# mx-mark/VideoTransformer-pytorch

Hardware: NVIDIA H100
Metric: clips/sec (BxTx3x224x224) TimeSformer-B fwd+bwd (higher is better)
Workload: dtype bf16

## Files before the change

### videotransformer_pytorch_b200/csrc/vt_attention_mma.cu

```cuda
#include "vt_attention_mma.cuh"

namespace vt {

constexpr int MT = 64;
constexpr int MMA_THREADS = 128;
constexpr float MMA_LOG2E = 1.4426950408889634f;
constexpr float MMA_LN2 = 0.6931471805599453f;

__device__ __forceinline__ void mma16816(float (&c)[4], uint32_t a0, uint32_t a1, uint32_t a2, uint32_t a3, uint32_t b0,
                                         uint32_t b1) {
  asm volatile(
      "mma.sync.aligned.m16n8k16.row.col.f32.bf16.bf16.f32 {%0,%1,%2,%3}, {%4,%5,%6,%7}, {%8,%9}, {%0,%1,%2,%3};"
      : "+f"(c[0]), "+f"(c[1]), "+f"(c[2]), "+f"(c[3])
      : "r"(a0), "r"(a1), "r"(a2), "r"(a3), "r"(b0), "r"(b1));
}
__device__ __forceinline__ uint32_t ld32(const __nv_bfloat16* p) { return *reinterpret_cast<const uint32_t*>(p); }
__device__ __forceinline__ uint32_t smem_addr(const void* p) { return static_cast<uint32_t>(__cvta_generic_to_shared(p)); }
template <int N>
__device__ __forceinline__ void zero(float (&x)[N][4]) {
#pragma unroll
  for (int i = 0; i < N; ++i) x[i][0] = x[i][1] = x[i][2] = x[i][3] = 0.f;
}

__device__ __forceinline__ void cp_async16(void* dst, const void* src, bool ok) {
  asm volatile("cp.async.cg.shared.global [%0], [%1], 16, %2;" ::"r"(smem_addr(dst)), "l"(src), "r"(ok ? 16 : 0) : "memory");
}
__device__ __forceinline__ void cp_async4(void* dst, const void* src, bool ok) {
  asm volatile("cp.async.ca.shared.global [%0], [%1], 4, %2;" ::"r"(smem_addr(dst)), "l"(src), "r"(ok ? 4 : 0) : "memory");
}
__device__ __forceinline__ void cp_async_commit() { asm volatile("cp.async.commit_group;" ::: "memory"); }
template <int N>
__device__ __forceinline__ void cp_async_wait() { asm volatile("cp.async.wait_group %0;" ::"n"(N) : "memory"); }

__device__ __forceinline__ void ldsm_x4(uint32_t (&r)[4], uint32_t a) {
  asm volatile("ldmatrix.sync.aligned.m8n8.x4.shared.b16 {%0,%1,%2,%3}, [%4];" : "=r"(r[0]), "=r"(r[1]), "=r"(r[2]), "=r"(r[3]) : "r"(a));
}
__device__ __forceinline__ void ldsm_x4_t(uint32_t (&r)[4], uint32_t a) {
  asm volatile("ldmatrix.sync.aligned.m8n8.x4.trans.shared.b16 {%0,%1,%2,%3}, [%4];" : "=r"(r[0]), "=r"(r[1]), "=r"(r[2]), "=r"(r[3]) : "r"(a));
}

template <int P>
__device__ __forceinline__ int lane_a(int lane) { return (lane & 15) * P + (lane >> 4) * 8; }
template <int P>
__device__ __forceinline__ int lane_b(int lane) { return ((lane & 7) + (lane >> 4) * 8) * P + ((lane >> 3) & 1) * 8; }

template <int HD>
struct PaddedTile {
  static constexpr int P = HD + 8;
  uint32_t base;
  int la, lb;
  __device__ __forceinline__ explicit PaddedTile(const __nv_bfloat16* t)
      : base(smem_addr(t)), la(2 * lane_a<P>(threadIdx.x & 31)), lb(2 * lane_b<P>(threadIdx.x & 31)) {}
  __device__ __forceinline__ uint32_t a(int r0, int c0) const { return base + (r0 * P + c0) * 2 + la; }
  __device__ __forceinline__ uint32_t b(int n0, int c0) const { return base + (n0 * P + c0) * 2 + lb; }
};

__device__ __forceinline__ int swz(int r, int c) { return r * 64 + ((c ^ (r & 7)) << 3); }
struct SwizzledTile {
  uint32_t base;
  int ar, ak, br, bk;
  __device__ __forceinline__ SwizzledTile(uint32_t operand, int r0) : base(operand + r0 * 128) {
    const int lane = threadIdx.x & 31;
    ar = (lane & 15) * 128; ak = (lane >> 4) ^ (lane & 7);
    br = ((lane & 7) + (lane >> 4) * 8) * 128; bk = ((lane >> 3) & 1) ^ (lane & 7);
  }
  __device__ __forceinline__ uint32_t a(int r0, int c0) const { return base + ar + r0 * 128 + (((c0 >> 3) ^ ak) << 4); }
  __device__ __forceinline__ uint32_t b(int n0, int c0) const { return base + br + n0 * 128 + (((c0 >> 3) ^ bk) << 4); }
};

template <int HD>
__device__ __forceinline__ void stage_rows(__nv_bfloat16* dst, const __nv_bfloat16* src, long long rs, int r0, int limit) {
#pragma unroll
  for (int i = threadIdx.x; i < MT * HD / 8; i += MMA_THREADS) {
    const int r = i / (HD / 8), c = (i % (HD / 8)) * 8;
    const bool ok = r0 + r < limit;
    cp_async16(dst + r * (HD + 8) + c, ok ? src + (long long)(r0 + r) * rs + c : src, ok);
  }
}
template <int HD, class DO2>
__device__ __forceinline__ float row_delta(bool ok, int half, DO2 dO2, const __nv_bfloat16* orow) {
  float d = 0.f;
  if (ok) {
#pragma unroll 4
    for (int c = half * (HD / 2); c < (half + 1) * (HD / 2); c += 2) {
      const float2 g = unpack_bf16x2(dO2(c));
      const float2 o = unpack_bf16x2(ld32(orow + c));
      d = fmaf(g.x, o.x, fmaf(g.y, o.y, d));
    }
  }
  return d + __shfl_xor_sync(0xffffffffu, d, 1);
}
template <int HD>
__device__ __forceinline__ void stage_row_stats(float* lse_s, float* del_s, const __nv_bfloat16* dOs, const __nv_bfloat16* orow,
                                                long long o_rs, const float* lrow, int r0, int limit, float* delta_out) {
  const int r = threadIdx.x >> 1, half = threadIdx.x & 1;
  const bool ok = r0 + r < limit;
  const __nv_bfloat16* g = dOs + r * (HD + 8);
  const float d = row_delta<HD>(ok, half, [=](int c) { return ld32(g + c); }, orow + r * o_rs);
  if (half == 0) {
    del_s[r] = d;
    lse_s[r] = ok ? lrow[r] * MMA_LOG2E : INFINITY;
    if (ok && delta_out) delta_out[r0 + r] = d;
  }
}


template <int KC, class Tile>
__device__ __forceinline__ void load_a(uint32_t (&f)[KC][4], const Tile& t, int r0) {
#pragma unroll
  for (int kc = 0; kc < KC; ++kc) ldsm_x4(f[kc], t.a(r0, kc * 16));
}

template <int HD>
struct FwdAcc {
  float o[HD / 8][4];
  float m0 = -INFINITY, m1 = -INFINITY, l0 = 0.f, l1 = 0.f;
  __device__ __forceinline__ FwdAcc() { zero(o); }
};

template <int HD, class Tile>
__device__ __forceinline__ void fwd_tile(FwdAcc<HD>& f, const uint32_t (&qa)[HD / 16][4], const Tile& K, const Tile& V, int k0,
                                         int N, float c) {
  constexpr int NB = HD / 8, KC = HD / 16;
  const int t = threadIdx.x & 3;
  float s[8][4];
  zero(s);
#pragma unroll
  for (int nb = 0; nb < 8; nb += 2) {
    if (k0 + nb * 8 >= N) break;
    const bool hi = k0 + nb * 8 + 8 < N;
#pragma unroll
    for (int kc = 0; kc < KC; ++kc) {
      uint32_t kf[4];
      ldsm_x4(kf, K.b(nb * 8, kc * 16));
      mma16816(s[nb], qa[kc][0], qa[kc][1], qa[kc][2], qa[kc][3], kf[0], kf[1]);
      if (hi) mma16816(s[nb + 1], qa[kc][0], qa[kc][1], qa[kc][2], qa[kc][3], kf[2], kf[3]);
    }
  }
  float mx0 = -INFINITY, mx1 = -INFINITY;
#pragma unroll
  for (int nb = 0; nb < 8; ++nb) {
#pragma unroll
    for (int e = 0; e < 4; ++e) {
      const int key = k0 + nb * 8 + 2 * t + (e & 1);
      const float v = key < N ? s[nb][e] * c : -INFINITY;
      s[nb][e] = v;
      if (e < 2) mx0 = fmaxf(mx0, v); else mx1 = fmaxf(mx1, v);
    }
  }
  mx0 = fmaxf(mx0, __shfl_xor_sync(0xffffffffu, mx0, 1)); mx0 = fmaxf(mx0, __shfl_xor_sync(0xffffffffu, mx0, 2));
  mx1 = fmaxf(mx1, __shfl_xor_sync(0xffffffffu, mx1, 1)); mx1 = fmaxf(mx1, __shfl_xor_sync(0xffffffffu, mx1, 2));
  const float mn0 = fmaxf(f.m0, mx0), mn1 = fmaxf(f.m1, mx1);
  const float corr0 = fast_exp2(f.m0 - mn0), corr1 = fast_exp2(f.m1 - mn1);
  f.l0 *= corr0; f.l1 *= corr1;
#pragma unroll
  for (int nb = 0; nb < NB; ++nb) { f.o[nb][0] *= corr0; f.o[nb][1] *= corr0; f.o[nb][2] *= corr1; f.o[nb][3] *= corr1; }
#pragma unroll
  for (int nb = 0; nb < 8; ++nb) {
    s[nb][0] = fast_exp2(s[nb][0] - mn0); s[nb][1] = fast_exp2(s[nb][1] - mn0);
    s[nb][2] = fast_exp2(s[nb][2] - mn1); s[nb][3] = fast_exp2(s[nb][3] - mn1);
    f.l0 += s[nb][0] + s[nb][1];
    f.l1 += s[nb][2] + s[nb][3];
  }
  f.m0 = mn0; f.m1 = mn1;
#pragma unroll
  for (int kc = 0; kc < 4; ++kc) {
    if (k0 + kc * 16 >= N) break;
    const uint32_t a0 = pack_bf16x2(s[2 * kc][0], s[2 * kc][1]), a1 = pack_bf16x2(s[2 * kc][2], s[2 * kc][3]);
    const uint32_t a2 = pack_bf16x2(s[2 * kc + 1][0], s[2 * kc + 1][1]), a3 = pack_bf16x2(s[2 * kc + 1][2], s[2 * kc + 1][3]);
#pragma unroll
    for (int nb = 0; nb < NB; nb += 2) {
      uint32_t vf[4];
      ldsm_x4_t(vf, V.a(kc * 16, nb * 8));
      mma16816(f.o[nb], a0, a1, a2, a3, vf[0], vf[1]);
      mma16816(f.o[nb + 1], a0, a1, a2, a3, vf[2], vf[3]);
    }
  }
}

template <int HD, bool LSE>
__device__ __forceinline__ void fwd_store(FwdAcc<HD>& f, const MmaAttn& p, int b, int h, int rb) {
  const int g = (threadIdx.x & 31) >> 2, t = threadIdx.x & 3;
  f.l0 += __shfl_xor_sync(0xffffffffu, f.l0, 1); f.l0 += __shfl_xor_sync(0xffffffffu, f.l0, 2);
  f.l1 += __shfl_xor_sync(0xffffffffu, f.l1, 1); f.l1 += __shfl_xor_sync(0xffffffffu, f.l1, 2);
  const float inv0 = 1.0f / f.l0, inv1 = 1.0f / f.l1;
  __nv_bfloat16* ob = p.o_out + b * p.o_bs + h * p.o_hs;
  const int r0 = rb + g, r1 = r0 + 8;
#pragma unroll
  for (int nb = 0; nb < HD / 8; ++nb) {
    if (r0 < p.Nq) *reinterpret_cast<uint32_t*>(ob + (long long)r0 * p.o_rs + nb * 8 + 2 * t) = pack_bf16x2(f.o[nb][0] * inv0, f.o[nb][1] * inv0);
    if (r1 < p.Nq) *reinterpret_cast<uint32_t*>(ob + (long long)r1 * p.o_rs + nb * 8 + 2 * t) = pack_bf16x2(f.o[nb][2] * inv1, f.o[nb][3] * inv1);
  }
  if (LSE && t == 0) {
    float* lse = p.lse + (long long)(b * p.H + h) * p.Nq;
    if (r0 < p.Nq) lse[r0] = (f.m0 + log2f(f.l0)) * MMA_LN2;
    if (r1 < p.Nq) lse[r1] = (f.m1 + log2f(f.l1)) * MMA_LN2;
  }
}

template <int HD, class Tile>
__device__ __forceinline__ void dq_tile(float (&dq)[HD / 8][4], const uint32_t (&qa)[HD / 16][4], const uint32_t (&da)[HD / 16][4],
                                        const Tile& K, const Tile& V, int k0, int N, float c, float lse0, float lse1, float del0, float del1) {
  constexpr int NB = HD / 8, KC = HD / 16;
  const int t = threadIdx.x & 3;
  float s[8][4], dpv[8][4];
  zero(s);
  zero(dpv);
#pragma unroll
  for (int nb = 0; nb < 8; nb += 2) {
    if (k0 + nb * 8 >= N) break;
    const bool hi = k0 + nb * 8 + 8 < N;
#pragma unroll
    for (int kc = 0; kc < KC; ++kc) {
      uint32_t kf[4], vf[4];
      ldsm_x4(kf, K.b(nb * 8, kc * 16));
      ldsm_x4(vf, V.b(nb * 8, kc * 16));
      mma16816(s[nb], qa[kc][0], qa[kc][1], qa[kc][2], qa[kc][3], kf[0], kf[1]);
      mma16816(dpv[nb], da[kc][0], da[kc][1], da[kc][2], da[kc][3], vf[0], vf[1]);
      if (hi) {
        mma16816(s[nb + 1], qa[kc][0], qa[kc][1], qa[kc][2], qa[kc][3], kf[2], kf[3]);
        mma16816(dpv[nb + 1], da[kc][0], da[kc][1], da[kc][2], da[kc][3], vf[2], vf[3]);
      }
    }
  }
#pragma unroll
  for (int nb = 0; nb < 8; ++nb) {
#pragma unroll
    for (int e = 0; e < 4; ++e) {
      const int key = k0 + nb * 8 + 2 * t + (e & 1);
      const float pr = key < N ? fast_exp2(s[nb][e] * c - (e < 2 ? lse0 : lse1)) : 0.f;
      s[nb][e] = pr * (dpv[nb][e] - (e < 2 ? del0 : del1));
    }
  }
#pragma unroll
  for (int kc = 0; kc < 4; ++kc) {
    if (k0 + kc * 16 >= N) break;
    const uint32_t a0 = pack_bf16x2(s[2 * kc][0], s[2 * kc][1]), a1 = pack_bf16x2(s[2 * kc][2], s[2 * kc][3]);
    const uint32_t a2 = pack_bf16x2(s[2 * kc + 1][0], s[2 * kc + 1][1]), a3 = pack_bf16x2(s[2 * kc + 1][2], s[2 * kc + 1][3]);
#pragma unroll
    for (int nb = 0; nb < NB; nb += 2) {
      uint32_t kf[4];
      ldsm_x4_t(kf, K.a(kc * 16, nb * 8));
      mma16816(dq[nb], a0, a1, a2, a3, kf[0], kf[1]);
      mma16816(dq[nb + 1], a0, a1, a2, a3, kf[2], kf[3]);
    }
  }
}

template <int HD>
__device__ __forceinline__ void dq_store(const float (&dq)[HD / 8][4], const MmaAttn& p, int b, int h, int rb) {
  const int g = (threadIdx.x & 31) >> 2, t = threadIdx.x & 3;
  __nv_bfloat16* dqb = p.dq + b * p.dq_bs + h * p.dq_hs;
  const int r0 = rb + g, r1 = r0 + 8;
#pragma unroll
  for (int nb = 0; nb < HD / 8; ++nb) {
    if (r0 < p.Nq)
      *reinterpret_cast<uint32_t*>(dqb + (long long)r0 * p.dq_rs + nb * 8 + 2 * t) = pack_bf16x2(dq[nb][0] * p.scale, dq[nb][1] * p.scale);
    if (r1 < p.Nq)
      *reinterpret_cast<uint32_t*>(dqb + (long long)r1 * p.dq_rs + nb * 8 + 2 * t) = pack_bf16x2(dq[nb][2] * p.scale, dq[nb][3] * p.scale);
  }
}

template <int HD, class Tile>
__device__ __forceinline__ void dkv_tile(float (&dk)[HD / 8][4], float (&dv)[HD / 8][4], const Tile& K, const Tile& V, int rb,
                                         const Tile& Q, const Tile& dO, int q0, int N, float c, const float* lse, const float* del) {
  constexpr int NB = HD / 8, KC = HD / 16;
  const int t = threadIdx.x & 3;
  float s[8][4], dpv[8][4];
  zero(s);
  zero(dpv);
#pragma unroll
  for (int kc = 0; kc < KC; ++kc) {
    uint32_t ka[4], va[4];
    ldsm_x4(ka, K.a(rb, kc * 16));
    ldsm_x4(va, V.a(rb, kc * 16));
#pragma unroll
    for (int nb = 0; nb < 8; nb += 2) {
      if (q0 + nb * 8 >= N) break;
      uint32_t qf[4], df[4];
      ldsm_x4(qf, Q.b(nb * 8, kc * 16));
      ldsm_x4(df, dO.b(nb * 8, kc * 16));
      mma16816(s[nb], ka[0], ka[1], ka[2], ka[3], qf[0], qf[1]);
      mma16816(dpv[nb], va[0], va[1], va[2], va[3], df[0], df[1]);
      if (q0 + nb * 8 + 8 < N) {
        mma16816(s[nb + 1], ka[0], ka[1], ka[2], ka[3], qf[2], qf[3]);
        mma16816(dpv[nb + 1], va[0], va[1], va[2], va[3], df[2], df[3]);
      }
    }
  }
#pragma unroll
  for (int nb = 0; nb < 8; ++nb) {
#pragma unroll
    for (int e = 0; e < 4; ++e) {
      const int qi = nb * 8 + 2 * t + (e & 1);
      const float pr = fast_exp2(s[nb][e] * c - lse[qi]);
      s[nb][e] = pr;
      dpv[nb][e] = pr * (dpv[nb][e] - del[qi]);
    }
  }
#pragma unroll
  for (int kc = 0; kc < 4; ++kc) {
    if (q0 + kc * 16 >= N) break;
    const uint32_t p0 = pack_bf16x2(s[2 * kc][0], s[2 * kc][1]), p1 = pack_bf16x2(s[2 * kc][2], s[2 * kc][3]);
    const uint32_t p2 = pack_bf16x2(s[2 * kc + 1][0], s[2 * kc + 1][1]), p3 = pack_bf16x2(s[2 * kc + 1][2], s[2 * kc + 1][3]);
    const uint32_t d0 = pack_bf16x2(dpv[2 * kc][0], dpv[2 * kc][1]), d1 = pack_bf16x2(dpv[2 * kc][2], dpv[2 * kc][3]);
    const uint32_t d2 = pack_bf16x2(dpv[2 * kc + 1][0], dpv[2 * kc + 1][1]), d3 = pack_bf16x2(dpv[2 * kc + 1][2], dpv[2 * kc + 1][3]);
#pragma unroll
    for (int nb = 0; nb < NB; nb += 2) {
      uint32_t gf[4], qf[4];
      ldsm_x4_t(gf, dO.a(kc * 16, nb * 8));
      ldsm_x4_t(qf, Q.a(kc * 16, nb * 8));
      mma16816(dv[nb], p0, p1, p2, p3, gf[0], gf[1]);
      mma16816(dv[nb + 1], p0, p1, p2, p3, gf[2], gf[3]);
      mma16816(dk[nb], d0, d1, d2, d3, qf[0], qf[1]);
      mma16816(dk[nb + 1], d0, d1, d2, d3, qf[2], qf[3]);
    }
  }
}

template <int HD>
__device__ __forceinline__ void dkv_store(const float (&dk)[HD / 8][4], const float (&dv)[HD / 8][4], const MmaAttn& p, int b, int h,
                                          int rb, bool f32) {
  const int g = (threadIdx.x & 31) >> 2, t = threadIdx.x & 3;
  const int r0 = rb + g, r1 = r0 + 8;
#pragma unroll
  for (int nb = 0; nb < HD / 8; ++nb) {
    const int col = nb * 8 + 2 * t;
    if (f32) {
      float* dkb = p.dk32 + (long long)(b * p.H + h) * p.Nk * HD;
      float* dvb = p.dv32 + (long long)(b * p.H + h) * p.Nk * HD;
      if (r0 < p.Nk) {
        *reinterpret_cast<float2*>(dkb + (long long)r0 * HD + col) = make_float2(dk[nb][0] * p.scale, dk[nb][1] * p.scale);
        *reinterpret_cast<float2*>(dvb + (long long)r0 * HD + col) = make_float2(dv[nb][0], dv[nb][1]);
      }
      if (r1 < p.Nk) {
        *reinterpret_cast<float2*>(dkb + (long long)r1 * HD + col) = make_float2(dk[nb][2] * p.scale, dk[nb][3] * p.scale);
        *reinterpret_cast<float2*>(dvb + (long long)r1 * HD + col) = make_float2(dv[nb][2], dv[nb][3]);
      }
    } else {
      __nv_bfloat16* dkb = p.dk16 + b * p.dk_bs + h * p.dk_hs;
      __nv_bfloat16* dvb = p.dv16 + b * p.dv_bs + h * p.dv_hs;
      if (r0 < p.Nk) {
        *reinterpret_cast<uint32_t*>(dkb + (long long)r0 * p.dk_rs + col) = pack_bf16x2(dk[nb][0] * p.scale, dk[nb][1] * p.scale);
        *reinterpret_cast<uint32_t*>(dvb + (long long)r0 * p.dv_rs + col) = pack_bf16x2(dv[nb][0], dv[nb][1]);
      }
      if (r1 < p.Nk) {
        *reinterpret_cast<uint32_t*>(dkb + (long long)r1 * p.dk_rs + col) = pack_bf16x2(dk[nb][2] * p.scale, dk[nb][3] * p.scale);
        *reinterpret_cast<uint32_t*>(dvb + (long long)r1 * p.dv_rs + col) = pack_bf16x2(dv[nb][2], dv[nb][3]);
      }
    }
  }
}

template <int HD, bool LSE>
__global__ void __launch_bounds__(MMA_THREADS) attn_mma_fwd_kernel(const MmaAttn p) {
  constexpr int TILE = MT * (HD + 8);
  extern __shared__ __align__(16) uint8_t mma_smem[];
  __nv_bfloat16* Qs = reinterpret_cast<__nv_bfloat16*>(mma_smem);
  __nv_bfloat16* ring = Qs + TILE;
  const int bh = blockIdx.y, b = bh / p.H, h = bh % p.H;
  const int q0 = blockIdx.x * MT, rb = (threadIdx.x >> 5) * 16;
  const bool active = q0 + rb < p.Nq;
  const __nv_bfloat16* kb = p.k + b * p.k_bs + h * p.k_hs;
  const __nv_bfloat16* vb = p.v + b * p.v_bs + h * p.v_hs;
  stage_rows<HD>(Qs, p.q + b * p.q_bs + h * p.q_hs, p.q_rs, q0, p.Nq);
  cp_async_commit();
  stage_rows<HD>(ring, kb, p.k_rs, 0, p.Nk);
  stage_rows<HD>(ring + TILE, vb, p.v_rs, 0, p.Nk);
  cp_async_commit();
  cp_async_wait<1>();
  __syncthreads();
  uint32_t qa[HD / 16][4];
  load_a(qa, PaddedTile<HD>(Qs), rb);
  FwdAcc<HD> f;
  const float c = p.scale * MMA_LOG2E;
  for (int k0 = 0, it = 0; k0 < p.Nk; k0 += MT, ++it) {
    cp_async_wait<0>();
    __syncthreads();
    if (k0 + MT < p.Nk) {
      __nv_bfloat16* nx = ring + ((it + 1) & 1) * 2 * TILE;
      stage_rows<HD>(nx, kb, p.k_rs, k0 + MT, p.Nk);
      stage_rows<HD>(nx + TILE, vb, p.v_rs, k0 + MT, p.Nk);
      cp_async_commit();
    }
    if (!active) continue;
    const __nv_bfloat16* Ks = ring + (it & 1) * 2 * TILE;
    fwd_tile<HD>(f, qa, PaddedTile<HD>(Ks), PaddedTile<HD>(Ks + TILE), k0, p.Nk, c);
  }
  if (active) fwd_store<HD, LSE>(f, p, b, h, q0 + rb);
}

template <int HD>
__global__ void __launch_bounds__(MMA_THREADS) attn_mma_dq_kernel(const MmaAttn p) {
  constexpr int TILE = MT * (HD + 8);
  extern __shared__ __align__(16) uint8_t mma_smem[];
  __nv_bfloat16* Qs = reinterpret_cast<__nv_bfloat16*>(mma_smem);
  __nv_bfloat16* dOs = Qs + TILE;
  __nv_bfloat16* ring = dOs + TILE;
  float* lse_s = reinterpret_cast<float*>(ring + 4 * TILE);
  float* del_s = lse_s + MT;
  const int bh = blockIdx.y, b = bh / p.H, h = bh % p.H;
  const int q0 = blockIdx.x * MT, g = (threadIdx.x & 31) >> 2, rb = (threadIdx.x >> 5) * 16;
  const bool active = q0 + rb < p.Nq;
  const __nv_bfloat16* kb = p.k + b * p.k_bs + h * p.k_hs;
  const __nv_bfloat16* vb = p.v + b * p.v_bs + h * p.v_hs;
  stage_rows<HD>(Qs, p.q + b * p.q_bs + h * p.q_hs, p.q_rs, q0, p.Nq);
  stage_rows<HD>(dOs, p.dout + b * p.o_bs + h * p.o_hs, p.o_rs, q0, p.Nq);
  cp_async_commit();
  stage_rows<HD>(ring, kb, p.k_rs, 0, p.Nk);
  stage_rows<HD>(ring + TILE, vb, p.v_rs, 0, p.Nk);
  cp_async_commit();
  cp_async_wait<1>();
  __syncthreads();
  stage_row_stats<HD>(lse_s, del_s, dOs, p.o + b * p.o_bs + h * p.o_hs + q0 * p.o_rs, p.o_rs,
                      p.lse + (long long)bh * p.Nq + q0, q0, p.Nq, p.delta ? p.delta + (long long)bh * p.Nq : nullptr);
  uint32_t qa[HD / 16][4], da[HD / 16][4];
  load_a(qa, PaddedTile<HD>(Qs), rb);
  load_a(da, PaddedTile<HD>(dOs), rb);
  __syncthreads();
  const float lse0 = lse_s[rb + g], lse1 = lse_s[rb + g + 8], del0 = del_s[rb + g], del1 = del_s[rb + g + 8];
  float dq[HD / 8][4];
  zero(dq);
  const float c = p.scale * MMA_LOG2E;
  for (int k0 = 0, it = 0; k0 < p.Nk; k0 += MT, ++it) {
    cp_async_wait<0>();
    __syncthreads();
    if (k0 + MT < p.Nk) {
      __nv_bfloat16* nx = ring + ((it + 1) & 1) * 2 * TILE;
      stage_rows<HD>(nx, kb, p.k_rs, k0 + MT, p.Nk);
      stage_rows<HD>(nx + TILE, vb, p.v_rs, k0 + MT, p.Nk);
      cp_async_commit();
    }
    if (!active) continue;
    const __nv_bfloat16* Ks = ring + (it & 1) * 2 * TILE;
    dq_tile<HD>(dq, qa, da, PaddedTile<HD>(Ks), PaddedTile<HD>(Ks + TILE), k0, p.Nk, c, lse0, lse1, del0, del1);
  }
  if (active) dq_store<HD>(dq, p, b, h, q0 + rb);
}

template <int HD>
__global__ void __launch_bounds__(MMA_THREADS, HD == 64 ? 3 : 1) attn_mma_dkv_kernel(const MmaAttn p) {
  constexpr int TILE = MT * (HD + 8);
  extern __shared__ __align__(16) uint8_t mma_smem[];
  __nv_bfloat16* Ks = reinterpret_cast<__nv_bfloat16*>(mma_smem);
  __nv_bfloat16* Vs = Ks + TILE;
  __nv_bfloat16* ring = Vs + TILE;
  float* lse_ring = reinterpret_cast<float*>(ring + 6 * TILE);
  float* lse_s = lse_ring + 2 * MT;
  float* del_s = lse_s + MT;
  const int bh = blockIdx.y, b = bh / p.H, h = bh % p.H;
  const int k0 = blockIdx.x * MT, rb = (threadIdx.x >> 5) * 16;
  const bool active = k0 + rb < p.Nk;
  const __nv_bfloat16* qb = p.q + b * p.q_bs + h * p.q_hs;
  const __nv_bfloat16* db = p.dout + b * p.o_bs + h * p.o_hs;
  const __nv_bfloat16* ob = p.o + b * p.o_bs + h * p.o_hs;
  const float* lse = p.lse + (long long)bh * p.Nq;
  auto stage_tile = [&](int st, int q0) {
    __nv_bfloat16* d = ring + st * 3 * TILE;
    stage_rows<HD>(d, qb, p.q_rs, q0, p.Nq);
    stage_rows<HD>(d + TILE, db, p.o_rs, q0, p.Nq);
    stage_rows<HD>(d + 2 * TILE, ob, p.o_rs, q0, p.Nq);
    if (threadIdx.x < MT) {
      const bool ok = q0 + (int)threadIdx.x < p.Nq;
      cp_async4(lse_ring + st * MT + threadIdx.x, ok ? lse + q0 + threadIdx.x : lse, ok);
    }
    cp_async_commit();
  };
  stage_rows<HD>(Ks, p.k + b * p.k_bs + h * p.k_hs, p.k_rs, k0, p.Nk);
  stage_rows<HD>(Vs, p.v + b * p.v_bs + h * p.v_hs, p.v_rs, k0, p.Nk);
  stage_tile(0, 0);
  float dk[HD / 8][4], dv[HD / 8][4];
  zero(dk);
  zero(dv);
  const float c = p.scale * MMA_LOG2E;
  for (int q0 = 0, it = 0; q0 < p.Nq; q0 += MT, ++it) {
    cp_async_wait<0>();
    __syncthreads();
    if (q0 + MT < p.Nq) stage_tile((it + 1) & 1, q0 + MT);
    const __nv_bfloat16* Qs = ring + (it & 1) * 3 * TILE;
    const __nv_bfloat16* dOs = Qs + TILE;
    stage_row_stats<HD>(lse_s, del_s, dOs, dOs + TILE, HD + 8, lse_ring + (it & 1) * MT, q0, p.Nq, nullptr);
    __syncthreads();
    if (!active) continue;
    dkv_tile<HD>(dk, dv, PaddedTile<HD>(Ks), PaddedTile<HD>(Vs), rb, PaddedTile<HD>(Qs), PaddedTile<HD>(dOs), q0, p.Nq, c,
                 lse_s, del_s);
  }
  if (active) dkv_store<HD>(dk, dv, p, b, h, k0 + rb, p.dk32 != nullptr);
}

constexpr int WHOLE_MAX_N = 256;
constexpr int WF_THREADS = 256;
constexpr int WB_THREADS = 192;

template <int THREADS>
__device__ __forceinline__ void stage_whole(__nv_bfloat16* dst, const __nv_bfloat16* src, long long rs, int r_begin, int r_end,
                                            int n) {
  for (int i = r_begin * 8 + threadIdx.x; i < r_end * 8; i += THREADS) {
    const int r = i >> 3, c = i & 7;
    const bool ok = r < n;
    cp_async16(dst + swz(r, c), ok ? src + (long long)r * rs + c * 8 : src, ok);
  }
}

template <bool LSE>
__global__ void __launch_bounds__(WF_THREADS, 2) attn_whole_fwd_kernel(const MmaAttn p) {
  constexpr int HD = 64, NW = WF_THREADS / 32;
  extern __shared__ __align__(16) uint8_t mma_smem[];
  const int N = p.Nq, R = (N + 15) & ~15, R0 = min(R, MT);
  __nv_bfloat16* Qs = reinterpret_cast<__nv_bfloat16*>(mma_smem);
  __nv_bfloat16* Ks = Qs + R * HD;
  __nv_bfloat16* Vs = Ks + R * HD;
  const int bh = blockIdx.x, b = bh / p.H, h = bh % p.H;
  const int warp = threadIdx.x >> 5;
  const __nv_bfloat16* kb = p.k + b * p.k_bs + h * p.k_hs;
  const __nv_bfloat16* vb = p.v + b * p.v_bs + h * p.v_hs;
  stage_whole<WF_THREADS>(Qs, p.q + b * p.q_bs + h * p.q_hs, p.q_rs, 0, R, N);
  stage_whole<WF_THREADS>(Ks, kb, p.k_rs, 0, R0, N);
  stage_whole<WF_THREADS>(Vs, vb, p.v_rs, 0, R0, N);
  cp_async_commit();
  stage_whole<WF_THREADS>(Ks, kb, p.k_rs, R0, R, N);
  stage_whole<WF_THREADS>(Vs, vb, p.v_rs, R0, R, N);
  cp_async_commit();
  cp_async_wait<1>();
  __syncthreads();
  const float c = p.scale * MMA_LOG2E;
  const int rounds = (R / 16 + NW - 1) / NW;
  for (int round = 0; round < rounds; ++round) {
    const int rb = (round * NW + warp) * 16;
    const bool active = rb < N;
    uint32_t qa[HD / 16][4];
    if (active) load_a(qa, SwizzledTile(smem_addr(Qs), 0), rb);
    FwdAcc<HD> f;
    for (int k0 = 0; k0 < N; k0 += MT) {
      if (round == 0 && k0 == MT) {
        cp_async_wait<0>();
        __syncthreads();
      }
      if (!active) continue;
      fwd_tile<HD>(f, qa, SwizzledTile(smem_addr(Ks), k0), SwizzledTile(smem_addr(Vs), k0), k0, N, c);
    }
    if (active) fwd_store<HD, LSE>(f, p, b, h, rb);
  }
}

struct WholeBwd {
  uint32_t Qs, Ks, Vs, dOs;
  const float *lse_s, *del_s;
  __device__ __forceinline__ WholeBwd(int N) {
    extern __shared__ __align__(16) uint8_t mma_smem[];
    const int R = (N + 15) & ~15, R64 = (N + MT - 1) & ~(MT - 1);
    Qs = smem_addr(mma_smem); Ks = Qs + R * 128; Vs = Ks + R * 128; dOs = Vs + R * 128;
    lse_s = reinterpret_cast<const float*>(mma_smem + 4 * R * 128);
    del_s = lse_s + R64;
  }
};

__device__ __forceinline__ void whole_dq_task(const MmaAttn& p, int rb) {
  const int N = p.Nq, g = (threadIdx.x & 31) >> 2;
  const WholeBwd w(N);
  uint32_t qa[4][4], da[4][4];
  load_a(qa, SwizzledTile(w.Qs, 0), rb);
  load_a(da, SwizzledTile(w.dOs, 0), rb);
  const float lse0 = w.lse_s[rb + g], lse1 = w.lse_s[rb + g + 8], del0 = w.del_s[rb + g], del1 = w.del_s[rb + g + 8];
  float dq[8][4];
  zero(dq);
  const float c = p.scale * MMA_LOG2E;
  for (int k0 = 0; k0 < N; k0 += MT)
    dq_tile<64>(dq, qa, da, SwizzledTile(w.Ks, k0), SwizzledTile(w.Vs, k0), k0, N, c, lse0, lse1, del0, del1);
  dq_store<64>(dq, p, blockIdx.x / p.H, blockIdx.x % p.H, rb);
}

__device__ __forceinline__ void whole_dkv_task(const MmaAttn& p, int rb) {
  const int N = p.Nq;
  const WholeBwd w(N);
  float dk[8][4], dv[8][4];
  zero(dk);
  zero(dv);
  const float c = p.scale * MMA_LOG2E;
  for (int q0 = 0; q0 < N; q0 += MT)
    dkv_tile<64>(dk, dv, SwizzledTile(w.Ks, 0), SwizzledTile(w.Vs, 0), rb, SwizzledTile(w.Qs, q0), SwizzledTile(w.dOs, q0), q0, N, c,
                 w.lse_s + q0, w.del_s + q0);
  dkv_store<64>(dk, dv, p, blockIdx.x / p.H, blockIdx.x % p.H, rb, false);
}

__global__ void __launch_bounds__(WB_THREADS, 2) attn_whole_bwd_kernel(const MmaAttn p) {
  constexpr int HD = 64;
  extern __shared__ __align__(16) uint8_t mma_smem[];
  __shared__ int next_task;
  const int N = p.Nq, R = (N + 15) & ~15, R64 = (N + MT - 1) & ~(MT - 1);
  __nv_bfloat16* Qs = reinterpret_cast<__nv_bfloat16*>(mma_smem);
  __nv_bfloat16* Ks = Qs + R * HD;
  __nv_bfloat16* Vs = Ks + R * HD;
  __nv_bfloat16* dOs = Vs + R * HD;
  float* lse_s = reinterpret_cast<float*>(dOs + R * HD);
  float* del_s = lse_s + R64;
  const int bh = blockIdx.x, b = bh / p.H, h = bh % p.H;
  const int lane = threadIdx.x & 31;
  stage_whole<WB_THREADS>(Qs, p.q + b * p.q_bs + h * p.q_hs, p.q_rs, 0, R, N);
  stage_whole<WB_THREADS>(Ks, p.k + b * p.k_bs + h * p.k_hs, p.k_rs, 0, R, N);
  stage_whole<WB_THREADS>(Vs, p.v + b * p.v_bs + h * p.v_hs, p.v_rs, 0, R, N);
  stage_whole<WB_THREADS>(dOs, p.dout + b * p.o_bs + h * p.o_hs, p.o_rs, 0, R, N);
  cp_async_commit();
  if (threadIdx.x == 0) next_task = 0;
  cp_async_wait<0>();
  __syncthreads();
  const __nv_bfloat16* ob = p.o + b * p.o_bs + h * p.o_hs;
  const float* lrow = p.lse + (long long)bh * N;
  for (int r0 = 0; r0 < R64; r0 += WB_THREADS / 2) {
    const int r = r0 + (threadIdx.x >> 1), half = threadIdx.x & 1;
    const bool ok = r < N;
    const float d = row_delta<HD>(ok, half, [=](int c) { return ld32(dOs + swz(r, c >> 3) + (c & 7)); }, ob + (long long)r * p.o_rs);
    if (half == 0 && r < R64) {
      del_s[r] = d;
      lse_s[r] = ok ? lrow[r] * MMA_LOG2E : INFINITY;
    }
  }
  __syncthreads();
  for (;;) {
    int task = 0;
    if (lane == 0) task = atomicAdd(&next_task, 1);
    task = __shfl_sync(0xffffffffu, task, 0) * 16;
    const int rows = (p.Nq + 15) & ~15;
    if (task >= 2 * rows) break;
    if (task < rows) whole_dkv_task(p, task);
    else whole_dq_task(p, task - rows);
  }
}

bool mma_layout_ok(const void* ptr, long long bs, long long hs, long long rs, int hd) {
  return ((uintptr_t)ptr & 15) == 0 && bs % 8 == 0 && hs % 8 == 0 && rs % 8 == 0 && (hs == hd || rs == hd);
}

template <int HD>
static constexpr int tile_bytes() { return MT * (HD + 8) * 2; }
template <int HD>
static constexpr int fwd_smem() { return 5 * tile_bytes<HD>(); }
template <int HD>
static constexpr int dq_smem() { return 6 * tile_bytes<HD>() + 2 * MT * 4; }
template <int HD>
static constexpr int dkv_smem() { return 8 * tile_bytes<HD>() + 4 * MT * 4; }

template <auto Kern>
static int launch(dim3 grid, int smem, const MmaAttn& a, cudaStream_t st, const char* what) {
  static bool done = false;
  if (!done) {
    cudaError_t e = cudaFuncSetAttribute(Kern, cudaFuncAttributeMaxDynamicSharedMemorySize, smem);
    VT_REQUIRE(e == cudaSuccess, "%s: smem attribute: %s", what, cudaGetErrorString(e));
    done = true;
  }
  Kern<<<grid, MMA_THREADS, smem, st>>>(a);
  return check_launch(what);
}

int attn_mma_fwd(const MmaAttn& a, int B, int hd, cudaStream_t st) {
  VT_REQUIRE(hd == 64 || hd == 96, "tensor-core attention: head dim %d unsupported (64 or 96)", hd);
  VT_REQUIRE((long long)B * a.H <= 65535, "tensor-core attention: B*H too large");
  const dim3 grid((a.Nq + MT - 1) / MT, B * a.H);
  const char* what = "attn_mma_fwd_kernel";
  if (hd == 64)
    return a.lse ? launch<attn_mma_fwd_kernel<64, true>>(grid, fwd_smem<64>(), a, st, what)
                 : launch<attn_mma_fwd_kernel<64, false>>(grid, fwd_smem<64>(), a, st, what);
  return a.lse ? launch<attn_mma_fwd_kernel<96, true>>(grid, fwd_smem<96>(), a, st, what)
               : launch<attn_mma_fwd_kernel<96, false>>(grid, fwd_smem<96>(), a, st, what);
}

int attn_mma_bwd(const MmaAttn& a, int B, int hd, cudaStream_t st) {
  VT_REQUIRE(hd == 64 || hd == 96, "tensor-core attention: head dim %d unsupported (64 or 96)", hd);
  VT_REQUIRE((long long)B * a.H <= 65535, "tensor-core attention: B*H too large");
  int rc;
  const dim3 gq((a.Nq + MT - 1) / MT, B * a.H), gk((a.Nk + MT - 1) / MT, B * a.H);
  if (hd == 64) {
    if ((rc = launch<attn_mma_dq_kernel<64>>(gq, dq_smem<64>(), a, st, "attn_mma_dq_kernel"))) return rc;
    return launch<attn_mma_dkv_kernel<64>>(gk, dkv_smem<64>(), a, st, "attn_mma_dkv_kernel");
  }
  if ((rc = launch<attn_mma_dq_kernel<96>>(gq, dq_smem<96>(), a, st, "attn_mma_dq_kernel"))) return rc;
  return launch<attn_mma_dkv_kernel<96>>(gk, dkv_smem<96>(), a, st, "attn_mma_dkv_kernel");
}

bool attn_whole_ok(const MmaAttn& a, int hd) {
  return hd == 64 && a.Nq == a.Nk && a.Nq >= 1 && a.Nq <= WHOLE_MAX_N && !a.dk32 && !a.delta;
}

static int whole_fwd_smem(int n) { return 3 * ((n + 15) & ~15) * 64 * 2; }
static int whole_bwd_smem(int n) { return 4 * ((n + 15) & ~15) * 64 * 2 + 2 * ((n + MT - 1) & ~(MT - 1)) * 4; }

template <auto Kern>
static int launch_whole(int problems, int threads, int smem, int smem_max, const MmaAttn& a, cudaStream_t st, const char* what) {
  static bool done = false;
  if (!done) {
    cudaError_t e = cudaFuncSetAttribute(Kern, cudaFuncAttributeMaxDynamicSharedMemorySize, smem_max);
    if (e == cudaSuccess)
      e = cudaFuncSetAttribute(Kern, cudaFuncAttributePreferredSharedMemoryCarveout, cudaSharedmemCarveoutMaxShared);
    VT_REQUIRE(e == cudaSuccess, "%s: smem attribute: %s", what, cudaGetErrorString(e));
    done = true;
  }
  Kern<<<problems, threads, smem, st>>>(a);
  return check_launch(what);
}

int attn_whole_fwd(const MmaAttn& a, int B, cudaStream_t st) {
  VT_REQUIRE(attn_whole_ok(a, 64), "attn_whole_fwd: unsupported operands (N=%d)", a.Nq);
  VT_REQUIRE((long long)B * a.H <= 65535, "tensor-core attention: B*H too large");
  const int smem = whole_fwd_smem(a.Nq), smax = whole_fwd_smem(WHOLE_MAX_N);
  return a.lse ? launch_whole<attn_whole_fwd_kernel<true>>(B * a.H, WF_THREADS, smem, smax, a, st, "attn_whole_fwd_kernel")
               : launch_whole<attn_whole_fwd_kernel<false>>(B * a.H, WF_THREADS, smem, smax, a, st, "attn_whole_fwd_kernel");
}

int attn_whole_bwd(const MmaAttn& a, int B, cudaStream_t st) {
  VT_REQUIRE(attn_whole_ok(a, 64), "attn_whole_bwd: unsupported operands (N=%d)", a.Nq);
  VT_REQUIRE((long long)B * a.H <= 65535, "tensor-core attention: B*H too large");
  return launch_whole<attn_whole_bwd_kernel>(B * a.H, WB_THREADS, whole_bwd_smem(a.Nq), whole_bwd_smem(WHOLE_MAX_N), a, st,
                                             "attn_whole_bwd_kernel");
}

}
```

Measured before the change: 270.3.

## Make whole-sequence attention forward persistent with double-buffered mbarrier-tracked loads

The whole-sequence forward kernel becomes persistent: the grid is sized to the SM count and each block runs several (batch, head) problems. Warps take 16-row tasks from a shared atomic counter, and two shared-memory slots are refilled with cp.async, with completion signalled through mbarriers. The next problem's Q/K/V load overlaps compute on the current one, and launch and tail costs shrink. In exchange the block grows to 512 threads with doubled shared memory and one block per SM, and it adds spin-waits and atomics.

```diff
diff --git a/videotransformer_pytorch_b200/csrc/vt_attention_mma.cu b/videotransformer_pytorch_b200/csrc/vt_attention_mma.cu
--- a/videotransformer_pytorch_b200/csrc/vt_attention_mma.cu
+++ b/videotransformer_pytorch_b200/csrc/vt_attention_mma.cu
@@ -1,4 +1,5 @@
 #include "vt_attention_mma.cuh"
+#include "vt_sm90.cuh"
 
 namespace vt {
 
@@ -489,57 +490,83 @@
 }
 
 constexpr int WHOLE_MAX_N = 256;
-constexpr int WF_THREADS = 256;
+constexpr int WF_THREADS = 512;
 constexpr int WB_THREADS = 192;
 
 template <int THREADS>
 __device__ __forceinline__ void stage_whole(__nv_bfloat16* dst, const __nv_bfloat16* src, long long rs, int r_begin, int r_end,
                                             int n) {
-  for (int i = r_begin * 8 + threadIdx.x; i < r_end * 8; i += THREADS) {
+  for (int i = r_begin * 8 + threadIdx.x % THREADS; i < r_end * 8; i += THREADS) {
     const int r = i >> 3, c = i & 7;
     const bool ok = r < n;
     cp_async16(dst + swz(r, c), ok ? src + (long long)r * rs + c * 8 : src, ok);
   }
 }
 
+struct WholeQueue {
+  uint64_t loaded[2];
+  int next;
+  int retired[2];
+};
+
+__device__ __forceinline__ void cp_async_mbar_arrive(uint64_t* bar) {
+  asm volatile("cp.async.mbarrier.arrive.noinc.shared::cta.b64 [%0];" ::"r"(smem_addr(bar)) : "memory");
+}
+
+__device__ __forceinline__ int whole_bh(int j) { return blockIdx.x + j * gridDim.x; }
+
+__device__ __forceinline__ void whole_fwd_load(const MmaAttn& p, WholeQueue& q, int j, int s) {
+  extern __shared__ __align__(16) uint8_t mma_smem[];
+  const int N = p.Nq, R = (N + 15) & ~15, bh = whole_bh(j), b = bh / p.H, h = bh % p.H;
+  __nv_bfloat16* Qs = reinterpret_cast<__nv_bfloat16*>(mma_smem) + s * 3 * R * 64;
+  stage_whole<32>(Qs, p.q + b * p.q_bs + h * p.q_hs, p.q_rs, 0, R, N);
+  stage_whole<32>(Qs + R * 64, p.k + b * p.k_bs + h * p.k_hs, p.k_rs, 0, R, N);
+  stage_whole<32>(Qs + 2 * R * 64, p.v + b * p.v_bs + h * p.v_hs, p.v_rs, 0, R, N);
+  cp_async_mbar_arrive(&q.loaded[s]);
+}
+
 template <bool LSE>
-__global__ void __launch_bounds__(WF_THREADS, 2) attn_whole_fwd_kernel(const MmaAttn p) {
-  constexpr int HD = 64, NW = WF_THREADS / 32;
+__global__ void __launch_bounds__(WF_THREADS, 1) attn_whole_fwd_kernel(const MmaAttn p, int problems) {
+  constexpr int HD = 64;
   extern __shared__ __align__(16) uint8_t mma_smem[];
-  const int N = p.Nq, R = (N + 15) & ~15, R0 = min(R, MT);
-  __nv_bfloat16* Qs = reinterpret_cast<__nv_bfloat16*>(mma_smem);
-  __nv_bfloat16* Ks = Qs + R * HD;
-  __nv_bfloat16* Vs = Ks + R * HD;
-  const int bh = blockIdx.x, b = bh / p.H, h = bh % p.H;
+  __shared__ WholeQueue q;
+  const int mine = (problems - (int)blockIdx.x + (int)gridDim.x - 1) / (int)gridDim.x, lane = threadIdx.x & 31;
+  if (threadIdx.x == 0) {
+    mbar_init(&q.loaded[0], 32);
+    mbar_init(&q.loaded[1], 32);
+    q.next = q.retired[0] = q.retired[1] = 0;
+  }
+  __syncthreads();
   const int warp = threadIdx.x >> 5;
-  const __nv_bfloat16* kb = p.k + b * p.k_bs + h * p.k_hs;
-  const __nv_bfloat16* vb = p.v + b * p.v_bs + h * p.v_hs;
-  stage_whole<WF_THREADS>(Qs, p.q + b * p.q_bs + h * p.q_hs, p.q_rs, 0, R, N);
-  stage_whole<WF_THREADS>(Ks, kb, p.k_rs, 0, R0, N);
-  stage_whole<WF_THREADS>(Vs, vb, p.v_rs, 0, R0, N);
-  cp_async_commit();
-  stage_whole<WF_THREADS>(Ks, kb, p.k_rs, R0, R, N);
-  stage_whole<WF_THREADS>(Vs, vb, p.v_rs, R0, R, N);
-  cp_async_commit();
-  cp_async_wait<1>();
-  __syncthreads();
+  if (warp < 2 && warp < mine) whole_fwd_load(p, q, warp, warp);
+  const int N = p.Nq, R = (N + 15) & ~15, T = R / 16;
   const float c = p.scale * MMA_LOG2E;
-  const int rounds = (R / 16 + NW - 1) / NW;
-  for (int round = 0; round < rounds; ++round) {
-    const int rb = (round * NW + warp) * 16;
-    const bool active = rb < N;
+  for (;;) {
+    int t = 0;
+    if (lane == 0) t = atomicAdd(&q.next, 1);
+    t = __shfl_sync(0xffffffffu, t, 0);
+    const int j = t / T, s = j & 1, use = j >> 1, rb = (t - j * T) * 16;
+    if (j >= mine) break;
+    if (lane == 0) {
+      const volatile int* retired = &q.retired[s];
+      while (*retired < use * T) __nanosleep(32);
+    }
+    __syncwarp();
+    mbar_wait(&q.loaded[s], use & 1);
+    const uint32_t Qs = smem_addr(mma_smem) + s * 3 * R * 128, Ks = Qs + R * 128, Vs = Ks + R * 128;
     uint32_t qa[HD / 16][4];
-    if (active) load_a(qa, SwizzledTile(smem_addr(Qs), 0), rb);
+    load_a(qa, SwizzledTile(Qs, 0), rb);
     FwdAcc<HD> f;
-    for (int k0 = 0; k0 < N; k0 += MT) {
-      if (round == 0 && k0 == MT) {
-        cp_async_wait<0>();
-        __syncthreads();
-      }
-      if (!active) continue;
-      fwd_tile<HD>(f, qa, SwizzledTile(smem_addr(Ks), k0), SwizzledTile(smem_addr(Vs), k0), k0, N, c);
-    }
-    if (active) fwd_store<HD, LSE>(f, p, b, h, rb);
+    for (int k0 = 0; k0 < N; k0 += MT) fwd_tile<HD>(f, qa, SwizzledTile(Ks, k0), SwizzledTile(Vs, k0), k0, N, c);
+    const int bh = whole_bh(j);
+    fwd_store<HD, LSE>(f, p, bh / p.H, bh % p.H, rb);
+    __syncwarp();
+    int last = 0;
+    if (lane == 0) {
+      __threadfence_block();
+      last = atomicAdd(&q.retired[s], 1) + 1 == (use + 1) * T;
+    }
+    if (__shfl_sync(0xffffffffu, last, 0) && j + 2 < mine) whole_fwd_load(p, q, j + 2, s);
   }
 }
 
@@ -684,8 +711,13 @@
 static int whole_fwd_smem(int n) { return 3 * ((n + 15) & ~15) * 64 * 2; }
 static int whole_bwd_smem(int n) { return 4 * ((n + 15) & ~15) * 64 * 2 + 2 * ((n + MT - 1) & ~(MT - 1)) * 4; }
 
-template <auto Kern>
-static int launch_whole(int problems, int threads, int smem, int smem_max, const MmaAttn& a, cudaStream_t st, const char* what) {
+static int whole_fwd_grid(int problems) {
+  const int sms = persistent_sm_count(), per = (problems + sms - 1) / sms;
+  return (problems + per - 1) / per;
+}
+
+template <auto Kern, class... Args>
+static int launch_whole(int grid, int threads, int smem, int smem_max, cudaStream_t st, const char* what, Args... args) {
   static bool done = false;
   if (!done) {
     cudaError_t e = cudaFuncSetAttribute(Kern, cudaFuncAttributeMaxDynamicSharedMemorySize, smem_max);
@@ -694,23 +726,23 @@
     VT_REQUIRE(e == cudaSuccess, "%s: smem attribute: %s", what, cudaGetErrorString(e));
     done = true;
   }
-  Kern<<<problems, threads, smem, st>>>(a);
+  Kern<<<grid, threads, smem, st>>>(args...);
   return check_launch(what);
 }
 
 int attn_whole_fwd(const MmaAttn& a, int B, cudaStream_t st) {
   VT_REQUIRE(attn_whole_ok(a, 64), "attn_whole_fwd: unsupported operands (N=%d)", a.Nq);
   VT_REQUIRE((long long)B * a.H <= 65535, "tensor-core attention: B*H too large");
-  const int smem = whole_fwd_smem(a.Nq), smax = whole_fwd_smem(WHOLE_MAX_N);
-  return a.lse ? launch_whole<attn_whole_fwd_kernel<true>>(B * a.H, WF_THREADS, smem, smax, a, st, "attn_whole_fwd_kernel")
-               : launch_whole<attn_whole_fwd_kernel<false>>(B * a.H, WF_THREADS, smem, smax, a, st, "attn_whole_fwd_kernel");
+  const int P = B * a.H, G = whole_fwd_grid(P), smem = 2 * whole_fwd_smem(a.Nq), smax = 2 * whole_fwd_smem(WHOLE_MAX_N);
+  return a.lse ? launch_whole<attn_whole_fwd_kernel<true>>(G, WF_THREADS, smem, smax, st, "attn_whole_fwd_kernel", a, P)
+               : launch_whole<attn_whole_fwd_kernel<false>>(G, WF_THREADS, smem, smax, st, "attn_whole_fwd_kernel", a, P);
 }
 
 int attn_whole_bwd(const MmaAttn& a, int B, cudaStream_t st) {
   VT_REQUIRE(attn_whole_ok(a, 64), "attn_whole_bwd: unsupported operands (N=%d)", a.Nq);
   VT_REQUIRE((long long)B * a.H <= 65535, "tensor-core attention: B*H too large");
-  return launch_whole<attn_whole_bwd_kernel>(B * a.H, WB_THREADS, whole_bwd_smem(a.Nq), whole_bwd_smem(WHOLE_MAX_N), a, st,
-                                             "attn_whole_bwd_kernel");
-}
-
-}
+  return launch_whole<attn_whole_bwd_kernel>(B * a.H, WB_THREADS, whole_bwd_smem(a.Nq), whole_bwd_smem(WHOLE_MAX_N), st,
+                                             "attn_whole_bwd_kernel", a);
+}
+
+}
```

Measured after the change: 271.7 (median of 6 runs). About the same (+0.5%).
